# SheffieldML/GPy

Hardware: AMD Instinct MI355X
Metric: exact-GP log_lik+grad iters/sec (higher is better)
Workload: dtype f64; 1 GPU; BASELINE configs[2]: matern52 ARD exact GP, one GPRegression.parameters_changed, N=16384 D=32 Dy=1 per GPU; N=16384, D=32, kernel=matern52, ARD=True, parallelism=replicas x1

## Files before the change

### gpy_amd/csrc/gemm.hip

```cpp
#include "gemm_tile.h"
#include "internal.h"

#define LDS_OPT_IN(kernel)                                                                              \
    do {                                                                                                \
        static bool done = false;                                                                       \
        if (!done) {                                                                                    \
            (void)hipFuncSetAttribute(reinterpret_cast<const void*>(kernel),                            \
                                      hipFuncAttributeMaxDynamicSharedMemorySize, GT_LDS_BYTES);        \
            done = true;                                                                                \
        }                                                                                               \
    } while (0)

#include <algorithm>
#include <cstdlib>
#include <vector>
#define env_int(name, dflt) diag_env_int(DIAG_ENV(name), dflt)
#define LB(NW) __launch_bounds__((NW) * 64, (NW) / 2)

template <int NW, bool PRE>
__global__ LB(NW) void k_update_nt(double* __restrict__ C, long ldc,
                                                      const double* __restrict__ A, long lda,
                                                      const double* __restrict__ B, long ldb, int K, int ntc,
                                                      int row0t, int col0t, int tri, long ntiles) {
    extern __shared__ __attribute__((aligned(16))) double smem[];
    for (long bid = blockIdx.x; bid < ntiles; bid += gridDim.x) {
        int ti, tj;
        if (tri) {
            ti = (int)((sqrtf(8.0f * (float)bid + 1.0f) - 1.0f) * 0.5f);
            while ((long)ti * (ti + 1) / 2 > bid) --ti;
            while ((long)(ti + 1) * (ti + 2) / 2 <= bid) ++ti;
            tj = (int)(bid - (long)ti * (ti + 1) / 2);
        } else {
            ti = (int)(bid / ntc);
            tj = (int)(bid - (long)ti * ntc);
            if (col0t + tj > row0t + ti) continue;
        }
        d4 acc[4][GTCfg<NW>::NI];
        double* Ct = C + (long)ti * NB * ldc + (long)tj * NB;
        if (PRE) {
            gt_load_buf<NW>(Ct, ldc, acc);
            gemm_tile_128<true, true, NW, true>(A + (long)ti * NB * lda, lda, B + (long)tj * NB * ldb, ldb, K, acc, smem);
            gt_store<0, NW>(Ct, ldc, acc);
        } else {
            gt_zero<NW>(acc);
            gemm_tile_128<true, true, NW>(A + (long)ti * NB * lda, lda, B + (long)tj * NB * ldb, ldb, K, acc, smem);
            gt_store<2, NW>(Ct, ldc, acc);
        }
    }
}

__global__ __launch_bounds__(256) void k_update_nt64(double* __restrict__ C, long ldc, const double* __restrict__ A, long lda,
                                                     const double* __restrict__ B, long ldb, int K, int ntc, int row0t,
                                                     int col0t, int tri) {
    extern __shared__ __attribute__((aligned(16))) double smem[];
    const long bid = blockIdx.x >> 2;
    const int qi = (blockIdx.x >> 1) & 1, qj = blockIdx.x & 1;
    int ti, tj;
    if (tri) {
        ti = (int)((sqrtf(8.0f * (float)bid + 1.0f) - 1.0f) * 0.5f);
        while ((long)ti * (ti + 1) / 2 > bid) --ti;
        while ((long)(ti + 1) * (ti + 2) / 2 <= bid) ++ti;
        tj = (int)(bid - (long)ti * (ti + 1) / 2);
    } else {
        ti = (int)(bid / ntc);
        tj = (int)(bid - (long)ti * ntc);
        if (col0t + tj > row0t + ti) return;
    }
    d4 acc[2][2];
    double* Ct = C + ((long)ti * NB + qi * 64) * ldc + (long)tj * NB + qj * 64;
    gt64_load(Ct, ldc, acc);
    gemm_tile_64_v3<true, true, true>(A + ((long)ti * NB + qi * 64) * lda, lda, B + ((long)tj * NB + qj * 64) * ldb, ldb, K,
                                      acc, smem);
    gt64_store<0>(Ct, ldc, acc);
}

bool update_nt_uses_64(int ntr, int ntc, int row0t, int col0t) {
    static const int upd64_max = env_int("UPD64_MAX", GEMM_DEFAULT_UPD64_MAX);
    const int tri = (row0t == col0t && ntr == ntc) ? 1 : 0;
    const long nblocks = tri ? (long)ntr * (ntr + 1) / 2 : (long)ntr * ntc;
    return nblocks <= upd64_max;
}

void launch_update_nt(hipStream_t st, double* C, long ldc, const double* A, long lda, const double* B, long ldb,
                      int K, int ntr, int ntc, int row0t, int col0t) {
    if (ntr <= 0 || ntc <= 0) return;
    const int tri = (row0t == col0t && ntr == ntc) ? 1 : 0;
    const long nblocks = tri ? (long)ntr * (ntr + 1) / 2 : (long)ntr * ntc;
    if (update_nt_uses_64(ntr, ntc, row0t, col0t)) {
        hipLaunchKernelGGL(k_update_nt64, dim3((unsigned)(4 * nblocks)), dim3(256), GT64_LDS_BYTES, st, C, ldc, A, lda, B, ldb,
                           K, ntc, row0t, col0t, tri);
        return;
    }
    LDS_OPT_IN((k_update_nt<4, true>));
    hipLaunchKernelGGL((k_update_nt<4, true>), dim3((unsigned)nblocks), dim3(256), GT_LDS_BYTES, st, C, ldc, A, lda, B, ldb, K,
                       ntc, row0t, col0t, tri, nblocks);
}

#ifdef MI355GP_DIAG
__global__ LB(4) void k_update_nt_queue(double* __restrict__ A, long ld, const UpdTask* __restrict__ tasks, int ntasks,
                                        int* __restrict__ counter) {
    extern __shared__ __attribute__((aligned(16))) double smem[];
    __shared__ long s_tile;
    for (;;) {
        __syncthreads();
        if (threadIdx.x == 0) s_tile = (long)atomicAdd(counter, 1);
        __syncthreads();
        long bid = s_tile;
        int q = 0;
        while (q < ntasks && bid >= tasks[q].ntiles) bid -= tasks[q++].ntiles;
        if (q >= ntasks) return;
        const UpdTask tk = tasks[q];
        int ti = (int)((sqrtf(8.0f * (float)bid + 1.0f) - 1.0f) * 0.5f);
        while ((long)ti * (ti + 1) / 2 > bid) --ti;
        while ((long)(ti + 1) * (ti + 2) / 2 <= bid) ++ti;
        const int tj = (int)(bid - (long)ti * (ti + 1) / 2);
        d4 acc[4][GTCfg<4>::NI];
        double* Ct = A + tk.c_off + (long)ti * NB * ld + (long)tj * NB;
        const double* P = A + tk.p_off;
        gt_load_buf<4>(Ct, ld, acc);
        gemm_tile_128<true, true, 4, true>(P + (long)ti * NB * ld, ld, P + (long)tj * NB * ld, ld, tk.K, acc, smem);
        gt_store<0, 4>(Ct, ld, acc);
    }
}

void launch_update_nt_queue(hipStream_t st, double* A, long ld, const UpdTask* tasks_dev, int ntasks, int* counter, int wgs) {
    LDS_OPT_IN(k_update_nt_queue);
    hipLaunchKernelGGL(k_update_nt_queue, dim3((unsigned)wgs), dim3(256), GT_LDS_BYTES, st, A, ld, tasks_dev, ntasks, counter);
}
#endif

__host__ __device__ __forceinline__ int trtri_rows_last(int nt, int nbt) {
    const int pairs = (nt + 2 * nbt - 1) / (2 * nbt), right0 = (2 * (pairs - 1) + 1) * nbt;
    const int rows = nt - right0;
    return rows < 0 ? 0 : (rows > nbt ? nbt : rows);
}
__host__ __device__ __forceinline__ long trtri_level_tiles(int nt, int nbt) {
    const int pairs = (nt + 2 * nbt - 1) / (2 * nbt);
    return (long)(pairs - 1) * nbt * nbt + (long)nbt * trtri_rows_last(nt, nbt);
}
template <int STAGE>
__device__ __forceinline__ void trtri_map(int bid, int nt, int nbt, int& p, int& ri, int& cj) {
    const int per = nbt * nbt, pairs = (nt + 2 * nbt - 1) / (2 * nbt), full = (pairs - 1) * per;
    if (bid < full) {
        p = bid / per;
        const int rem = bid - p * per;
        if (STAGE == 1) {
            cj = rem / nbt;
            ri = rem - cj * nbt;
        } else {
            ri = nbt - 1 - rem / nbt;
            cj = rem % nbt;
        }
    } else {
        p = pairs - 1;
        const int rem = bid - full, rows = trtri_rows_last(nt, nbt);
        if (STAGE == 1) {
            cj = rem / rows;
            ri = rem - cj * rows;
        } else {
            ri = rows - 1 - rem / nbt;
            cj = rem % nbt;
        }
    }
}

template <int STAGE, int NW>
__device__ __forceinline__ void trtri_stage_tile(int bid, const double* __restrict__ L, double* __restrict__ X,
                                                 double* __restrict__ T, long ld, int nt, int nbt, double* smem) {
    int p, ri, cj;
    trtri_map<STAGE>(bid, nt, nbt, p, ri, cj);
    const int left0 = 2 * p * nbt, right0 = left0 + nbt;
    const int ti = right0 + ri, tj = left0 + cj;
    if (ti >= nt) return;
    d4 acc[4][GTCfg<NW>::NI];
// ... 462 lines not shown
```

### gpy_amd/csrc/gemm_tile.h

```cpp
#pragma once
#include "common.h"

#define GT_LDS_BYTES 73728

template <int NW>
struct GTCfg {
    static_assert(NW == 4, "the tile kernels run 4-wave workgroups");
    static constexpr int NTHR = NW * 64;
    static constexpr int NI = 4;
    static constexpr int WCOLS = NI * 16;
    static constexpr int WPR = 128 / WCOLS;
};

template <bool AK, bool BK, bool NEGA = false>
__device__ __forceinline__ void gemm_tile_128_v3(const double* __restrict__ A, long lda, const double* __restrict__ B,
                                                 long ldb, int K, d4 (&acc)[4][4], double* smem);

template <bool AK, bool BK, int NW, bool NEGA = false>
__device__ __forceinline__ void gemm_tile_128(const double* __restrict__ A, long lda,
                                              const double* __restrict__ B, long ldb, int K,
                                              d4 (&acc)[4][GTCfg<NW>::NI], double* smem) {
    gemm_tile_128_v3<AK, BK, NEGA>(A, lda, B, ldb, K, acc, smem);
}

template <int NW>
__device__ __forceinline__ void gt_zero(d4 (&acc)[4][GTCfg<NW>::NI]) {
#pragma unroll
    for (int mi = 0; mi < 4; ++mi)
#pragma unroll
        for (int ni = 0; ni < GTCfg<NW>::NI; ++ni) acc[mi][ni] = (d4){0.0, 0.0, 0.0, 0.0};
}

template <int NW>
__device__ __forceinline__ double* gt_cbase(double* C, long ldc) {
    const int t = threadIdx.x, lane = t & 63, w = t >> 6, wr = w / GTCfg<NW>::WPR, wc = w % GTCfg<NW>::WPR;
    return C + (long)(wr * 64 + (lane >> 4)) * ldc + wc * GTCfg<NW>::WCOLS + (lane & 15);
}

template <int NW>
__device__ __forceinline__ void gt_load_buf(const double* Ct, long ldc, d4 (&acc)[4][GTCfg<NW>::NI]) {
    typedef unsigned int u2 __attribute__((ext_vector_type(2)));
    const int t = threadIdx.x, lane = t & 63, w = t >> 6, wr = w / GTCfg<NW>::WPR, wc = w % GTCfg<NW>::WPR;
    __amdgpu_buffer_rsrc_t rs = __builtin_amdgcn_make_buffer_rsrc(const_cast<double*>(Ct), 0, 0x7fffffff, 0x00020000);
    const int ldb = (int)ldc * 8;
    const int voff = (wr * 64 + (lane >> 4)) * ldb + (wc * GTCfg<NW>::WCOLS + (lane & 15)) * 8;
#pragma unroll
    for (int mi = 0; mi < 4; ++mi)
#pragma unroll
        for (int r = 0; r < 4; ++r) {
            const int soff = (mi * 16 + 4 * r) * ldb;
#pragma unroll
            for (int ni = 0; ni < GTCfg<NW>::NI; ++ni) {
                const u2 v = __builtin_amdgcn_raw_buffer_load_b64(rs, voff + ni * 128, soff, 0);
                acc[mi][ni][r] = __builtin_bit_cast(double, v);
            }
        }
}

template <int NW>
__device__ __forceinline__ void gt_load_neg(const double* __restrict__ C, long ldc, d4 (&acc)[4][GTCfg<NW>::NI]) {
    const double* base = gt_cbase<NW>(const_cast<double*>(C), ldc);
#pragma unroll
    for (int mi = 0; mi < 4; ++mi)
#pragma unroll
        for (int ni = 0; ni < GTCfg<NW>::NI; ++ni)
#pragma unroll
            for (int r = 0; r < 4; ++r) acc[mi][ni][r] = -base[(long)(mi * 16 + 4 * r) * ldc + ni * 16];
}

template <int MODE, int NW>
__device__ __forceinline__ void gt_store(double* __restrict__ C, long ldc, const d4 (&acc)[4][GTCfg<NW>::NI],
                                         double alpha = 1.0, double beta = 0.0) {
    constexpr int NI = GTCfg<NW>::NI;
    double* base = gt_cbase<NW>(C, ldc);
#pragma unroll
    for (int mi = 0; mi < 4; ++mi) {
        double old[NI][4];
        if (MODE >= 2) {
#pragma unroll
            for (int ni = 0; ni < NI; ++ni)
#pragma unroll
                for (int r = 0; r < 4; ++r) old[ni][r] = base[(long)(mi * 16 + 4 * r) * ldc + ni * 16];
        }
#pragma unroll
        for (int ni = 0; ni < NI; ++ni)
#pragma unroll
            for (int r = 0; r < 4; ++r) {
                double* p = base + (long)(mi * 16 + 4 * r) * ldc + ni * 16;
                const double v = acc[mi][ni][r];
                if (MODE == 0) *p = v;
                else if (MODE == 1) *p = -v;
                else if (MODE == 2) *p = old[ni][r] - v;
                else *p = alpha * v + beta * old[ni][r];
            }
    }
}

#define GT3_SMN 132
#define GT3_OP 2176
#define GT3_LDS_BYTES (2 * 2 * GT3_OP * 8)

__device__ __forceinline__ int gt3_h(int r) { return ((r >> 1) & 7) ^ ((((r & 15) >= 4) && ((r & 15) <= 11)) ? 2 : 0); }

template <bool KC>
__device__ __forceinline__ void gt3_src_offsets(long ld, int lane, int w, int (&voff)[4]) {
#pragma unroll
    for (int ii = 0; ii < 4; ++ii) {
        const int i = 4 * w + ii;
        if (KC) {
            const int row = 8 * i + (lane >> 3), g = (lane & 7) ^ gt3_h(row);
            voff[ii] = (int)((row * ld + 2 * g) * 8);
        } else {
            voff[ii] = (int)((i * ld + 2 * lane) * 8);
        }
    }
}

template <bool KC>
__device__ __forceinline__ void gt3_issue(__amdgpu_buffer_rsrc_t rs, const int (&voff)[4], int soff, double* sdst, int w) {
#pragma unroll
    for (int ii = 0; ii < 4; ++ii) {
        const int i = 4 * w + ii;
        double* d = KC ? sdst + i * 128 : sdst + i * GT3_SMN;
        __builtin_amdgcn_raw_ptr_buffer_load_lds(rs, d, 16, voff[ii], soff, 0, 0);
    }
}

template <bool AK, bool BK, bool NEGA>
__device__ __forceinline__ void gemm_tile_128_v3(const double* __restrict__ A, long lda,
                                                 const double* __restrict__ B, long ldb, int K, d4 (&acc)[4][4],
                                                 double* smem) {
    const int t = threadIdx.x, lane = t & 63, w = t >> 6, wr = w >> 1, wc = w & 1;
    const int nk = K / 16;
    const int arow = wr * 64 + (lane & 15), bcol = wc * 64 + (lane & 15), kq = lane >> 4;
    auto rsrc = [](const double* p) {
        return __builtin_amdgcn_make_buffer_rsrc(const_cast<double*>(p), 0, 0x7fffffff, 0x00020000);
    };
    int va[4], vb[4];
    gt3_src_offsets<AK>(lda, lane, w, va);
    gt3_src_offsets<BK>(ldb, lane, w, vb);
    const long sa = AK ? 16 : 16 * lda, sb = BK ? 16 : 16 * ldb;
    int fa0[4], fb0[4];
#pragma unroll
    for (int mi = 0; mi < 4; ++mi) {
        const int r = arow + mi * 16, c = bcol + mi * 16;
        fa0[mi] = AK ? r * 16 : r;
        fb0[mi] = BK ? c * 16 : c;
    }
    const int ha = gt3_h(arow), hb = gt3_h(bcol);
    gt3_issue<AK>(rsrc(A), va, 0, smem, w);
    gt3_issue<BK>(rsrc(B), vb, 0, smem + GT3_OP, w);
    __builtin_amdgcn_s_waitcnt(0x0F70);
    __syncthreads();
    for (int kt = 0; kt < nk; ++kt) {
        const int cur = kt & 1;
        if (kt + 1 < nk) {
            double* nxt = smem + (cur ^ 1) * 2 * GT3_OP;
            gt3_issue<AK>(rsrc(A + (kt + 1) * sa), va, 0, nxt, w);
            gt3_issue<BK>(rsrc(B + (kt + 1) * sb), vb, 0, nxt + GT3_OP, w);
        }
        const double* a_s = smem + cur * 2 * GT3_OP;
        const double* b_s = a_s + GT3_OP;
#pragma unroll
        for (int e = 0; e < 2; ++e) {
            d2 af[4], bf[4];
#pragma unroll
            for (int mi = 0; mi < 4; ++mi) {
                if (AK) af[mi] = *reinterpret_cast<const d2*>(a_s + fa0[mi] + 2 * ((2 * kq + e) ^ ha));
                else af[mi] = (d2){a_s[(4 * kq + 2 * e) * GT3_SMN + fa0[mi]], a_s[(4 * kq + 2 * e + 1) * GT3_SMN + fa0[mi]]};
            }
#pragma unroll
            for (int ni = 0; ni < 4; ++ni) {
                if (BK) bf[ni] = *reinterpret_cast<const d2*>(b_s + fb0[ni] + 2 * ((2 * kq + e) ^ hb));
                else bf[ni] = (d2){b_s[(4 * kq + 2 * e) * GT3_SMN + fb0[ni]], b_s[(4 * kq + 2 * e + 1) * GT3_SMN + fb0[ni]]};
            }
#pragma unroll
            for (int s = 0; s < 2; ++s)
#pragma unroll
                for (int mi = 0; mi < 4; ++mi)
#pragma unroll
                    for (int ni = 0; ni < 4; ++ni)
                        acc[mi][ni] = mfma_f64(NEGA ? -af[mi][s] : af[mi][s], bf[ni][s], acc[mi][ni]);
        }
        __builtin_amdgcn_s_waitcnt(0x0F70);
        __syncthreads();
    }
}


template <bool AK, bool BK, bool NEGA>
__device__ __forceinline__ void gemm_tile_128_v3_multi(const double* const* __restrict__ Atab, long aoff, long lda,
                                                       const double* const* __restrict__ Btab, long boff, long ldb,
                                                       int k0, int k1, int slabs, d4 (&acc)[4][4], double* smem) {
    const int t = threadIdx.x, lane = t & 63, w = t >> 6, wr = w >> 1, wc = w & 1;
    const int nk = (k1 - k0) * slabs;
    const int arow = wr * 64 + (lane & 15), bcol = wc * 64 + (lane & 15), kq = lane >> 4;
    auto rsrc = [](const double* p) {
        return __builtin_amdgcn_make_buffer_rsrc(const_cast<double*>(p), 0, 0x7fffffff, 0x00020000);
    };
    int va[4], vb[4];
    gt3_src_offsets<AK>(lda, lane, w, va);
    gt3_src_offsets<BK>(ldb, lane, w, vb);
    const long sa = AK ? 16 : 16 * lda, sb = BK ? 16 : 16 * ldb;
    int fa0[4], fb0[4];
#pragma unroll
    for (int mi = 0; mi < 4; ++mi) {
        const int r = arow + mi * 16, c = bcol + mi * 16;
        fa0[mi] = AK ? r * 16 : r;
        fb0[mi] = BK ? c * 16 : c;
    }
    const int ha = gt3_h(arow), hb = gt3_h(bcol);
    int pk = k0, ps = 0;
    const double* Ab = Atab[pk] + aoff;
    const double* Bb = Btab[pk] + boff;
    gt3_issue<AK>(rsrc(Ab), va, 0, smem, w);
    gt3_issue<BK>(rsrc(Bb), vb, 0, smem + GT3_OP, w);
    __builtin_amdgcn_s_waitcnt(0x0F70);
    __syncthreads();
    for (int kt = 0; kt < nk; ++kt) {
        const int cur = kt & 1;
        if (kt + 1 < nk) {
            if (++ps == slabs) {
                ps = 0;
                ++pk;
                Ab = Atab[pk] + aoff;
                Bb = Btab[pk] + boff;
            }
            double* nxt = smem + (cur ^ 1) * 2 * GT3_OP;
            gt3_issue<AK>(rsrc(Ab + ps * sa), va, 0, nxt, w);
            gt3_issue<BK>(rsrc(Bb + ps * sb), vb, 0, nxt + GT3_OP, w);
        }
        const double* a_s = smem + cur * 2 * GT3_OP;
        const double* b_s = a_s + GT3_OP;
#pragma unroll
        for (int e = 0; e < 2; ++e) {
            d2 af[4], bf[4];
#pragma unroll
            for (int mi = 0; mi < 4; ++mi) {
                if (AK) af[mi] = *reinterpret_cast<const d2*>(a_s + fa0[mi] + 2 * ((2 * kq + e) ^ ha));
                else af[mi] = (d2){a_s[(4 * kq + 2 * e) * GT3_SMN + fa0[mi]], a_s[(4 * kq + 2 * e + 1) * GT3_SMN + fa0[mi]]};
            }
#pragma unroll
            for (int ni = 0; ni < 4; ++ni) {
                if (BK) bf[ni] = *reinterpret_cast<const d2*>(b_s + fb0[ni] + 2 * ((2 * kq + e) ^ hb));
                else bf[ni] = (d2){b_s[(4 * kq + 2 * e) * GT3_SMN + fb0[ni]], b_s[(4 * kq + 2 * e + 1) * GT3_SMN + fb0[ni]]};
            }
#pragma unroll
            for (int s = 0; s < 2; ++s)
#pragma unroll
                for (int mi = 0; mi < 4; ++mi)
#pragma unroll
                    for (int ni = 0; ni < 4; ++ni)
                        acc[mi][ni] = mfma_f64(NEGA ? -af[mi][s] : af[mi][s], bf[ni][s], acc[mi][ni]);
        }
        __builtin_amdgcn_s_waitcnt(0x0F70);
        __syncthreads();
    }
}

#define GT64_OP 1088
#define GT64_PAIR 136
#define GT64_LDS_BYTES (2 * 2 * GT64_OP * 8)

template <bool KC>
__device__ __forceinline__ void gt64_src_offsets(long ld, int lane, int w, int (&voff)[2]) {
#pragma unroll
    for (int ii = 0; ii < 2; ++ii) {
        const int i = 2 * w + ii;
        if (KC) {
            const int row = 8 * i + (lane >> 3), g = (lane & 7) ^ gt3_h(row);
            voff[ii] = (int)((row * ld + 2 * g) * 8);
        } else {
            voff[ii] = (int)(((2 * i + (lane >> 5)) * ld + 2 * (lane & 31)) * 8);
        }
    }
}

template <bool KC>
__device__ __forceinline__ void gt64_issue(__amdgpu_buffer_rsrc_t rs, const int (&voff)[2], double* sdst, int w) {
#pragma unroll
    for (int ii = 0; ii < 2; ++ii) {
        const int i = 2 * w + ii;
        double* d = KC ? sdst + i * 128 : sdst + i * GT64_PAIR;
        __builtin_amdgcn_raw_ptr_buffer_load_lds(rs, d, 16, voff[ii], 0, 0, 0);
    }
}

template <bool AK, bool BK, bool NEGA = false>
__device__ __forceinline__ void gemm_tile_64_v3(const double* __restrict__ A, long lda, const double* __restrict__ B,
                                                long ldb, int K, d4 (&acc)[2][2], double* smem) {
    const int t = threadIdx.x, lane = t & 63, w = t >> 6, wr = w >> 1, wc = w & 1;
    const int nk = K / 16;
    const int arow = wr * 32 + (lane & 15), bcol = wc * 32 + (lane & 15), kq = lane >> 4;
    auto rsrc = [](const double* p) {
        return __builtin_amdgcn_make_buffer_rsrc(const_cast<double*>(p), 0, 0x7fffffff, 0x00020000);
    };
    int va[2], vb[2];
    gt64_src_offsets<AK>(lda, lane, w, va);
    gt64_src_offsets<BK>(ldb, lane, w, vb);
    const long sa = AK ? 16 : 16 * lda, sb = BK ? 16 : 16 * ldb;
    int fa0[2], fb0[2];
#pragma unroll
    for (int mi = 0; mi < 2; ++mi) {
        const int r = arow + mi * 16, c = bcol + mi * 16;
        fa0[mi] = AK ? r * 16 : r;
        fb0[mi] = BK ? c * 16 : c;
    }
    const int ha = gt3_h(arow), hb = gt3_h(bcol);
    gt64_issue<AK>(rsrc(A), va, smem, w);
    gt64_issue<BK>(rsrc(B), vb, smem + GT64_OP, w);
    __builtin_amdgcn_s_waitcnt(0x0F70);
    __syncthreads();
    for (int kt = 0; kt < nk; ++kt) {
        const int cur = kt & 1;
        if (kt + 1 < nk) {
            double* nxt = smem + (cur ^ 1) * 2 * GT64_OP;
            gt64_issue<AK>(rsrc(A + (kt + 1) * sa), va, nxt, w);
            gt64_issue<BK>(rsrc(B + (kt + 1) * sb), vb, nxt + GT64_OP, w);
        }
        const double* a_s = smem + cur * 2 * GT64_OP;
        const double* b_s = a_s + GT64_OP;
#pragma unroll
        for (int e = 0; e < 2; ++e) {
            d2 af[2], bf[2];
#pragma unroll
            for (int mi = 0; mi < 2; ++mi) {
                if (AK) af[mi] = *reinterpret_cast<const d2*>(a_s + fa0[mi] + 2 * ((2 * kq + e) ^ ha));
                else af[mi] = (d2){a_s[(2 * kq + e) * GT64_PAIR + fa0[mi]], a_s[(2 * kq + e) * GT64_PAIR + 64 + fa0[mi]]};
            }
#pragma unroll
            for (int ni = 0; ni < 2; ++ni) {
                if (BK) bf[ni] = *reinterpret_cast<const d2*>(b_s + fb0[ni] + 2 * ((2 * kq + e) ^ hb));
                else bf[ni] = (d2){b_s[(2 * kq + e) * GT64_PAIR + fb0[ni]], b_s[(2 * kq + e) * GT64_PAIR + 64 + fb0[ni]]};
            }
#pragma unroll
            for (int s = 0; s < 2; ++s)
#pragma unroll
                for (int mi = 0; mi < 2; ++mi)
#pragma unroll
                    for (int ni = 0; ni < 2; ++ni)
                        acc[mi][ni] = mfma_f64(NEGA ? -af[mi][s] : af[mi][s], bf[ni][s], acc[mi][ni]);
        }
        __builtin_amdgcn_s_waitcnt(0x0F70);
        __syncthreads();
    }
}

__device__ __forceinline__ void gt64_zero(d4 (&acc)[2][2]) {
#pragma unroll
    for (int mi = 0; mi < 2; ++mi)
#pragma unroll
        for (int ni = 0; ni < 2; ++ni) acc[mi][ni] = (d4){0.0, 0.0, 0.0, 0.0};
}

__device__ __forceinline__ void gt64_load(const double* __restrict__ C, long ldc, d4 (&acc)[2][2]) {
    const int t = threadIdx.x, lane = t & 63, w = t >> 6, wr = w >> 1, wc = w & 1;
    const double* base = C + (long)(wr * 32 + (lane >> 4)) * ldc + wc * 32 + (lane & 15);
#pragma unroll
    for (int mi = 0; mi < 2; ++mi)
#pragma unroll
        for (int ni = 0; ni < 2; ++ni)
#pragma unroll
            for (int r = 0; r < 4; ++r) acc[mi][ni][r] = base[(long)(mi * 16 + 4 * r) * ldc + ni * 16];
}

template <int MODE>
__device__ __forceinline__ void gt64_store(double* __restrict__ C, long ldc, const d4 (&acc)[2][2]) {
    const int t = threadIdx.x, lane = t & 63, w = t >> 6, wr = w >> 1, wc = w & 1;
    double* base = C + (long)(wr * 32 + (lane >> 4)) * ldc + wc * 32 + (lane & 15);
#pragma unroll
    for (int mi = 0; mi < 2; ++mi)
#pragma unroll
        for (int ni = 0; ni < 2; ++ni)
#pragma unroll
            for (int r = 0; r < 4; ++r) base[(long)(mi * 16 + 4 * r) * ldc + ni * 16] = (MODE == 1) ? -acc[mi][ni][r] : acc[mi][ni][r];
}
```

### gpy_amd/csrc/grid.hip

```cpp
#include <dlfcn.h>

#include <cmath>
#include <cstdlib>
#include <cstring>
#include <functional>
#include <string>
#include <vector>

#include "../../include/mi355gp.h"
#include "../../include/mi355gp_debug.h"
#include "gemm_tile.h"
#include "internal.h"
#include "parts.h"

#define LOG_2_PI 1.8378770664093454836

#include <rccl/rccl.h>
static_assert(sizeof(ncclUniqueId) == 128, "mi355gp_grid_unique_id hands out 128-byte ids");
ncclResult_t ipcGetUniqueId(ncclUniqueId* id);
ncclResult_t ipcCommInitRank(ncclComm_t* out, int nranks, ncclUniqueId id, int rank);
ncclResult_t ipcCommSplit(ncclComm_t parent, int color, int key, ncclComm_t* out, ncclConfig_t* cfg);
ncclResult_t ipcCommDestroy(ncclComm_t comm);
ncclResult_t ipcBroadcast(const void* send, void* recv, size_t count, ncclDataType_t type, int root, ncclComm_t comm, hipStream_t st);
ncclResult_t ipcAllReduce(const void* send, void* recv, size_t count, ncclDataType_t type, ncclRedOp_t op, ncclComm_t comm, hipStream_t st);
// ... 136 lines not shown
    const int ntr = (int)(M / NB), ntc = (int)(N / NB);
    hipLaunchKernelGGL((k_grid_gemm<AK, BK>), dim3((unsigned)(ntr * ntc)), dim3(256), GT_LDS_BYTES, st, C, ldc, c_tm,
                       a.p, a.ld, a.tm, b.p, b.ld, b.tm, (int)K, ntc, (int)(nb / NB), nb, mode, pd);
}

#define GRID_ROWTAB_MAX 960
struct GridRowTab {
    int n;
    int pre[GRID_ROWTAB_MAX + 1];
};
template <bool AK, bool BK, int MODE>
__global__ __launch_bounds__(256, 2) void k_grid_gemm_multi(double* __restrict__ C, long ldc,
                                                            const double* const* __restrict__ Atab,
                                                            const double* const* __restrict__ Btab, int k0, int k1,
                                                            int ti0, int tj0, int ntc, int q, long nb, int kpred,
                                                            GridPred pd, long ldo, int tm, GridRowTab rt) {
    extern __shared__ __attribute__((aligned(16))) double smem[];
    int ti, tj;
    if (tm == 2) {
        const int bid = blockIdx.x;
        ti = (int)((sqrtf(8.0f * (float)bid + 1.0f) - 1.0f) * 0.5f);
        while ((long)ti * (ti + 1) / 2 > bid) --ti;
        while ((long)(ti + 1) * (ti + 2) / 2 <= bid) ++ti;
        tj = bid - (int)((long)ti * (ti + 1) / 2);
    } else if (rt.n > 0) {
        const int qq = q * q, p = (int)(blockIdx.x / qq), sub = (int)(blockIdx.x % qq);
        int lo = 0, hi = rt.n - 1;
        while (lo < hi) {
            const int mid = (lo + hi + 1) >> 1;
            if (rt.pre[mid] <= p) lo = mid;
            else hi = mid - 1;
        }
        ti = ti0 + lo * q + sub / q;
        tj = tj0 + (p - rt.pre[lo]) * q + sub % q;
    } else {
        ti = ti0 + blockIdx.x / ntc;
        tj = tj0 + blockIdx.x % ntc;
    }
    const int I = (ti / q) * pd.Pr + pd.pr, J = (tj / q) * pd.Pc + pd.pc;
    if (pd.on && J > I) return;
    int ks = k0;
    if (kpred >= 1 && J > ks) ks = J;
    if (kpred >= 2 && I > ks) ks = I;
    double* Ct = C + (long)ti * NB * ldc + (long)tj * NB;
    d4 acc[4][4];
    if (ks >= k1) {
        if (MODE == 0) {
            gt_zero<4>(acc);
            gt_store<0, 4>(Ct, ldc, acc);
        }
        return;
    }
    if (MODE == 0) gt_zero<4>(acc);
    else gt_load_buf<4>(Ct, ldc, acc);
    const long aoff = AK ? (long)ti * NB * ldo : (tm == 1 ? (long)(ti / q) * nb * nb + (long)(ti % q) * NB : (long)ti * NB);
    const long boff = BK ? (long)tj * NB * ldo : (tm == 1 ? (long)(tj / q) * nb * nb + (long)(tj % q) * NB : (long)tj * NB);
    gemm_tile_128_v3_multi<AK, BK, MODE == 2>(Atab, aoff, ldo, Btab, boff, ldo, ks, k1, (int)(nb / 16), acc, smem);
    gt_store<0, 4>(Ct, ldc, acc);
}

template <bool AK, bool BK, int MODE>
static void grid_gemm_multi(hipStream_t st, double* C, long ldc, const double* const* Atab, const double* const* Btab,
                            int k0, int k1, int ti0, int ti1, int tj0, int tj1, long nb, int kpred, GridPred pd,
                            long ldo = 0, int tm = 1) {
    if (ti1 <= ti0 || tj1 <= tj0 || k1 <= k0) return;
    static bool opted = false;
    if (!opted) {
        (void)hipFuncSetAttribute(reinterpret_cast<const void*>(k_grid_gemm_multi<AK, BK, MODE>),
                                  hipFuncAttributeMaxDynamicSharedMemorySize, GT_LDS_BYTES);
        opted = true;
    }
    const int q = (int)(nb / NB), ntr = (ti1 - ti0) * q, ntc = (tj1 - tj0) * q;
    long nblk = (tm == 2) ? (long)ntr * (ntr + 1) / 2 : (long)ntr * ntc;
    GridRowTab rt;
    rt.n = 0;
    if (pd.on && tm != 2 && ti1 - ti0 <= GRID_ROWTAB_MAX) {
        long tot = 0;
        int first = -1, last = -1;
        for (int li = ti0; li < ti1; ++li) {
            const long I = (long)li * pd.Pr + pd.pr;
            long m = (I >= pd.pc) ? (I - pd.pc) / pd.Pc + 1 : 0;
            long c = m - tj0;
            if (c < 0) c = 0;
            if (c > tj1 - tj0) c = tj1 - tj0;
            if (c > 0) {
                if (first < 0) first = li;
                last = li;
            }
            if (first >= 0) rt.pre[li - first] = (int)tot;
            tot += c;
        }
        if (tot == 0) return;
        rt.n = last - first + 1;
        rt.pre[rt.n] = (int)tot;
        ti0 = first;
        nblk = tot * q * q;
    }
    hipLaunchKernelGGL((k_grid_gemm_multi<AK, BK, MODE>), dim3((unsigned)nblk), dim3(256), GT_LDS_BYTES, st, C, ldc,
                       Atab, Btab, k0, k1, ti0 * q, tj0 * q, ntc, q, nb, kpred, pd, ldo ? ldo : nb, tm, rt);
}

__global__ void k_grid_fix_diag(double* __restrict__ A, long ld, long nb, long n, int ndiag,
                                const int* __restrict__ dl_r, const int* __restrict__ dl_c,
                                const int* __restrict__ dg, const double* __restrict__ noise, long noise_len,
                                double jit) {
    const long idx = (long)blockIdx.x * blockDim.x + threadIdx.x;
    if (idx >= (long)ndiag * nb) return;
    const int d = (int)(idx / nb);
    const long e = idx % nb, g = (long)dg[d] * nb + e;
    double* p = A + ((long)dl_r[d] * nb + e) * ld + (long)dl_c[d] * nb + e;
    if (g < n) *p += noise[noise_len > 1 ? g : 0] + jit;
// ... 1316 lines not shown
```

### gpy_amd/csrc/persist.hip

```cpp
#include <atomic>
#include <cstdlib>
#include <vector>

#include "chain_dev.h"
#include "gemm_tile.h"
#include "internal.h"

#define PS_NEARD 2
#define PS_MAXNT 64
#define PS_MAXT 48
#define PS_STAGE_CHUNKS 14
#define PS_STAGE_DOUBLES (PS_STAGE_CHUNKS * 128)
#define PS_LDS_BYTES ((44 * TSZ + 4 * PS_STAGE_DOUBLES) * 8)
#define PS_TIMEOUT_TICKS 50000000LL
#define PS_ARRIVE_TICKS 100000LL
#define PS_ARRIVE_ABORT (1 << 30)

#define PS_DCNT 0
#define PS_ABORT 1
#define PS_ARRIVE 2
#define PS_CNT 16
#define PS_SUB (16 + PS_MAXNT)
#define PS_DIA (16 + 2 * PS_MAXNT)
#define PS_HA (16 + 3 * PS_MAXNT)
// ... 605 lines not shown
                if (s_prog[s] >= 0 && s_wait[s] && s_cnt[nt] >= s_tk[s] + 1) {
                    pick = s; pi = s_ti[s]; pk = s_tk[s];
                    pj0 = pj1 = (pi == pk) ? pi - 1 : ((split && pi == pk + 1 && pi >= 2) ? pk - 1 : pk);
                    ptrsm = 1;
                    break;
                }
            }
        for (int o = 0; o < nmine && pick < 0; ++o) {
            const int s = s_order[o];
            const int p = s_prog[s];
            if (p == -1) continue;
            if (hot && (s_tk[s] > hotk || s_ti[s] > hoti)) continue;
            const int i = s_ti[s], k = s_tk[s];
            if (p == -2) {
                if (s_cnt[i - 1] >= i - 1 && s_pre[i]) { pick = s; pi = i; pk = i - 1; pj0 = i - 2; pj1 = i - 1; pfin = 1; break; }
                continue;
            }
            const int limit = (i == k) ? i - 1 : ((split && i == k + 1 && i >= 2) ? k - 1 : k);
            if (s_wait[s]) {
                if (s_cnt[nt] >= k + 1) { pick = s; pi = i; pk = k; pj0 = pj1 = limit; ptrsm = 1; break; }
                continue;
            }
            int jmax = s_cnt[i] < s_cnt[k] ? s_cnt[i] : s_cnt[k];
            if (jmax > limit) jmax = limit;
            if (jmax > p || p == limit) {
                pick = s; pi = i; pk = k; pj0 = p;
                pj1 = (jmax > p + kcap) ? p + kcap : (jmax > p ? jmax : p);
                ptrsm = (pj1 == limit && i >= k + 2 && s_cnt[nt] >= k + 1) ? 1 : 0;
                break;
            }
        }
        if (pick < 0) {
            if (t == 0) {
                if (idle0 == 0) idle0 = wall_clock64();
                else if (wall_clock64() - idle0 > PS_TIMEOUT_TICKS) st_flag(sync + PS_ABORT, 1);
                if (me >= own.H + own.Hh) __builtin_amdgcn_s_sleep(8);
            }
            __syncthreads();
            continue;
        }
        idle0 = 0;
        const bool subdiag = (pi == pk + 1);
        const int limit = (pi == pk) ? pi - 1 : ((split && subdiag && pi >= 2 && !pfin) ? pk - 1 : pk);
        const bool general = pi >= pk + 2;
        double* Ct = A + (long)pi * NB * ld + (long)pk * NB;
        long long* dn = (dbg && pi - pk <= 2 && (pj1 == limit)) ? dbg + 8 * nt + 4 * (3 * pi + (pi - pk)) : nullptr;
        if (dn && t == 0) dn[0] = wall_clock64();
        long long* df = (dbg && pi - pk == 3 && pj1 == limit) ? dbg + 20 * nt + 12 * pi : nullptr;
        if (df && t == 0 && pj1 > pj0) df[0] = wall_clock64();
        const bool pre = (pj1 == limit && split && subdiag && pi >= 2 && !pfin);
        const bool handover = (pj1 == limit && !general && !pre);
        if (pj1 > pj0 || (handover && subdiag)) {
            d4 acc[4][4];
            gt_load_buf<4>(Ct, ld, acc);
            if (pj1 > pj0)
                gemm_tile_128<true, true, 4, true>(A + (long)pi * NB * ld + (long)pj0 * NB, ld,
                                                   A + (long)pk * NB * ld + (long)pj0 * NB, ld, (pj1 - pj0) * NB, acc, sm);
            if (handover || subdiag) {
                __syncthreads();
                stage_put_acc(sm, acc);
                __syncthreads();
                if (handover && subdiag) stage_store_chain_order<256>(sm, hs + (long)pi * (NB * NB), t);
                else stage_store_coherent<256>(sm, Ct, ld, t);
            } else {
                gt_store<0, 4>(Ct, ld, acc);
            }
        }
        if (dn && t == 0) dn[1] = wall_clock64();
        if (df && t == 0 && pj1 > pj0) df[1] = wall_clock64();
        if (handover) {
            drain_stores();
            __syncthreads();
            if (t == 0) {
                st_flag(sync + ((pi == pk) ? PS_DIA : PS_SUB) + pi, 1);
                if (dn) dn[2] = wall_clock64();
                s_prog[pick] = -1;
            }
            --left;
        } else if (pre) {
            drain_stores();
            __syncthreads();
            if (t == 0) {
                st_flag(sync + PS_PRE + pi, 1);
                s_prog[pick] = -1;
            }
            --left;
        } else if (pj1 == limit && !ptrsm) {
            drain_stores();
            __syncthreads();
            if (t == 0) { s_prog[pick] = pj1; s_wait[pick] = 1; }
        } else if (ptrsm) {
            drain_stores();
            __syncthreads();
            if (df && t == 0) df[2] = wall_clock64();
            trsm_stage_L(A, ld, (long)pk * NB, dinv_all + (long)pk * 8 * 256, sm);
            __syncthreads();
            if (df && t == 0) df[3] = wall_clock64();
            {
                d4 Y0[8], Y1[8];
                trsm_strip2_regs(A, ld, (long)pk * NB, (long)pi * NB + 16 * w, sm, lane, Y0, Y1);
                __syncthreads();
                if (df && t == 0) df[4] = wall_clock64();
                stage_put_strips(sm, w, Y0, Y1, lane);
            }
            __syncthreads();
            stage_store_coherent<256>(sm, Ct, ld, t);
            drain_stores();
            __syncthreads();
            const bool more = split && pi == pk + 2;
            if (t == 0) {
// ... 76 lines not shown
        if (t < nt) h_cnt[t] = ld_flag(sync + PS_CNT + t);
        if (t == 64) h_cnt[nt] = ld_flag(sync + PS_DCNT);
        if (t == 65) h_cnt[nt + 1] = ld_flag(sync + PS_ABORT);
        if (t >= 128 && t < 128 + nt) h_pre[t - 128] = ld_flag(sync + PS_PRE + t - 128);
        if (t == 0) __builtin_amdgcn_fence(__ATOMIC_ACQUIRE, "agent");
        __syncthreads();
        if (h_cnt[nt + 1] != 0) return;
        const int dc = h_cnt[nt];
        bool hot = false;
        if (nreserve >= 0)
            for (int s = 0; s < nmine; ++s) hot = hot || (h_stage[s] != 3 && own.half_row(q, s) <= dc + nreserve);
        int pick = -1, pi = 0, pj0 = 0, pj1 = 0, act = 0;
        for (int s = 0; s < nmine && pick < 0; ++s) {
            const int st = h_stage[s];
            if (st == 3) continue;
            const int i = own.half_row(q, s), k = i - 2;
            if (hot && i > dc + nreserve) continue;
            if (st == 2) {
                if (h_cnt[i - 1] >= i - 1 && h_pre[i] != 0) { pick = s; pi = i; act = 3; }
                continue;
            }
            if (st == 1) {
                if (dc >= k + 1) { pick = s; pi = i; act = 2; }
                continue;
            }
            const int p = h_prog[s];
            if (p >= k) {
                pick = s; pi = i; act = (dc >= k + 1) ? 2 : 0;
                if (act == 0) { pick = -1; if (t == 0) h_stage[s] = 1; }
                continue;
            }
            int jmax = h_cnt[i] < h_cnt[k] ? h_cnt[i] : h_cnt[k];
            if (jmax > k) jmax = k;
            if (jmax > p) { pick = s; pi = i; act = 1; pj0 = p; pj1 = (jmax > p + kcap) ? p + kcap : jmax; }
        }
        if (pick < 0) {
            if (t == 0) {
                if (idle0 == 0) idle0 = wall_clock64();
                else if (wall_clock64() - idle0 > PS_TIMEOUT_TICKS) st_flag(sync + PS_ABORT, 1);
            }
            __syncthreads();
            continue;
        }
        idle0 = 0;
        const int pk = pi - 2;
        const long r0 = (long)pi * NB + 64 * h;
        long long* dn2 = (dbg && h == 0) ? dbg + 8 * nt + 4 * (3 * pi + 2) : nullptr;
        long long* dn1 = (dbg && h == 0) ? dbg + 8 * nt + 4 * (3 * pi + 1) : nullptr;
        if (act == 1) {
#pragma unroll 1
            for (int qc = 0; qc < 2; ++qc) {
                double* Cq = A + r0 * ld + (long)pk * NB + 64 * qc;
                d4 acc[2][2];
                gt64_load(Cq, ld, acc);
                gemm_tile_64_v3<true, true, true>(A + r0 * ld + (long)pj0 * NB, ld, A + ((long)pk * NB + 64 * qc) * ld + (long)pj0 * NB, ld,
                                                  (pj1 - pj0) * NB, acc, sm);
                gt64_store<0>(Cq, ld, acc);
            }
            __syncthreads();
            if (t == 0) {
                h_prog[pick] = pj1;
                if (pj1 >= pk) h_stage[pick] = 1;
            }
        } else if (act == 2) {
            if (dn2 && t == 0) dn2[0] = wall_clock64();
            drain_stores();
            __syncthreads();
            trsm_stage_L(A, ld, (long)pk * NB, dinv_all + (long)pk * 8 * 256, sm);
            __syncthreads();
            {
                const int fi = lane & 15, fk = lane >> 4;
                const double* Pa = A + (r0 + 16 * w + fi) * ld + (long)pk * NB;
                d4 P[8], Y[8];
#pragma unroll
                for (int jb = 0; jb < 8; ++jb)
#pragma unroll
                    for (int r = 0; r < 4; ++r) P[jb][r] = Pa[jb * 16 + fk + 4 * r];
                trsm_strip_core(P, Y, [sm](int jb, int k) { return sm + tix_sl(jb, k) * TSZ; }, [sm](int jb) { return sm + (28 + jb) * TSZ; },
                                lane);
                if (dn2 && t == 0) dn2[1] = wall_clock64();
                half_put_strip(img, w, Y, lane);
            }
            __syncthreads();
            half_store_coherent(img, A + r0 * ld + (long)pk * NB, ld, t);
            drain_stores();
            __syncthreads();
            if (t == 0) {
                if (__hip_atomic_fetch_add(sync + PS_HA + pi, 1, __ATOMIC_RELAXED, __HIP_MEMORY_SCOPE_AGENT) == 1)
                    st_flag(sync + PS_CNT + pi, pk + 1);
                if (dn2) dn2[2] = wall_clock64();
                h_stage[pick] = 2;
            }
        } else {
            if (dn1 && t == 0) dn1[0] = wall_clock64();
#pragma unroll 1
            for (int qc = 0; qc < 2; ++qc) {
                const double* Cq = A + r0 * ld + (long)(pi - 1) * NB + 64 * qc;
                d4 acc[2][2];
                gt64_load(Cq, ld, acc);
                gemm_tile_64_v3<true, true, true>(A + r0 * ld + (long)pk * NB, ld, A + ((long)(pi - 1) * NB + 64 * qc) * ld + (long)pk * NB, ld,
                                                  NB, acc, sm);
                half_put_acc(img, acc, qc);
            }
            __syncthreads();
            if (dn1 && t == 0) dn1[1] = wall_clock64();
            half_store_chain_order(img, hs + (long)pi * (NB * NB), h, t);
            drain_stores();
            __syncthreads();
            if (t == 0) {
                if (__hip_atomic_fetch_add(sync + PS_HB + pi, 1, __ATOMIC_RELAXED, __HIP_MEMORY_SCOPE_AGENT) == 1)
                    st_flag(sync + PS_SUB + pi, 1);
                if (dn1) dn1[2] = wall_clock64();
                h_stage[pick] = 3;
            }
            --left;
        }
        __syncthreads();
    }
}

__global__ __launch_bounds__(512, 1) void k_potrf_persist(double* __restrict__ A, long ld, int nt,
                                                          double* __restrict__ dinv_all, double* __restrict__ logsum,
                                                          int* __restrict__ info, int* __restrict__ sync, int kcap,
                                                          double* __restrict__ hs, long long* __restrict__ dbg, int test, int tune) {
    extern __shared__ __attribute__((aligned(16))) double sm[];
    if (!ps_arrive(sync, info, test == 1 ? 1 : 0)) return;
    if (test == 2 && blockIdx.x == 0) {
        if (threadIdx.x == 0) {
            st_flag(sync + PS_ABORT, 1);
            atomicMax(info, PS_ABORT_INFO);
        }
        return;
    }
    if (blockIdx.x == 0) {
        chain_workgroup(A, ld, nt, dinv_all, logsum, info, sync, hs, dbg);
        if (threadIdx.x == 0 && ld_flag(sync + PS_ABORT) != 0) atomicMax(info, PS_ABORT_INFO);
    } else {
        const int split = (tune & 4) ? 0 : 1, neard = ps_neard(tune), hdiv = ((tune >> 8) & 0xff) ? ((tune >> 8) & 0xff) : ps_hdiv(nt);
        const int nreserve = (tune & 32) ? -1 : (((tune >> 16) & 7) ? ((tune >> 16) & 7) : 3);
        const int halves = ps_halves(nt, tune);
        int H, Hh, nnear;
        ps_near_split(nt, (int)gridDim.x - 1, neard, hdiv, halves, &H, &Hh, &nnear);
        const int me = (int)blockIdx.x - 1;
        if (me >= H && me < H + Hh)
            half_workgroup(A, ld, nt, dinv_all, sync, kcap, hs, dbg, neard, hdiv, nreserve, halves, sm);
        else
            worker_workgroup(A, ld, nt, dinv_all, sync, kcap, hs, dbg, split, neard, hdiv, (tune & 1) ? 0 : 1, (tune & 2) ? 0 : 1,
                             (tune & 8) ? -1 : ((tune & 16) ? 1 : 0), nreserve,
                             ((tune >> 20) & 1) ? 1 : (((tune >> 21) & 1) ? 0 : ps_far_rowmajor(nt)), halves, sm);
    }
}

int persist_box_verdict(int set) {
    static std::atomic<int> votes[2] = {{0}, {0}};
// ... 170 lines not shown
```

Baseline: 13.89 iters/s.

## Software-pipeline LDS fragment loads and hoist negation out of MFMA inner loop

The 128 and 64 GEMM tile kernels now load the next k-half's fragments from LDS while the MFMAs for the current half run, with sched_barriers fixing the order. Global-to-LDS prefetch moves two stages ahead, into the buffer just consumed. The NEGA per-MFMA negation of A fragments is dropped; callers instead negate C on load and store with a negating mode (or negate the accumulator explicitly), so the inner loop is pure MFMA. This adds register pressure from the double fragment sets and risks correctness if any store mode or buffer reuse is mismatched.

After: 14.00 iters/s (median of 6 runs). No clear change (+0.8%).

```diff
diff --git a/gpy_amd/csrc/gemm.hip b/gpy_amd/csrc/gemm.hip
--- a/gpy_amd/csrc/gemm.hip
+++ b/gpy_amd/csrc/gemm.hip
@@ -38,9 +38,9 @@
         d4 acc[4][GTCfg<NW>::NI];
         double* Ct = C + (long)ti * NB * ldc + (long)tj * NB;
         if (PRE) {
-            gt_load_buf<NW>(Ct, ldc, acc);
-            gemm_tile_128<true, true, NW, true>(A + (long)ti * NB * lda, lda, B + (long)tj * NB * ldb, ldb, K, acc, smem);
-            gt_store<0, NW>(Ct, ldc, acc);
+            gt_load_buf<NW, true>(Ct, ldc, acc);
+            gemm_tile_128<true, true, NW>(A + (long)ti * NB * lda, lda, B + (long)tj * NB * ldb, ldb, K, acc, smem);
+            gt_store<1, NW>(Ct, ldc, acc);
         } else {
             gt_zero<NW>(acc);
             gemm_tile_128<true, true, NW>(A + (long)ti * NB * lda, lda, B + (long)tj * NB * ldb, ldb, K, acc, smem);
@@ -68,10 +68,9 @@
     }
     d4 acc[2][2];
     double* Ct = C + ((long)ti * NB + qi * 64) * ldc + (long)tj * NB + qj * 64;
-    gt64_load(Ct, ldc, acc);
-    gemm_tile_64_v3<true, true, true>(A + ((long)ti * NB + qi * 64) * lda, lda, B + ((long)tj * NB + qj * 64) * ldb, ldb, K,
-                                      acc, smem);
-    gt64_store<0>(Ct, ldc, acc);
+    gt64_load<true>(Ct, ldc, acc);
+    gemm_tile_64_v3<true, true>(A + ((long)ti * NB + qi * 64) * lda, lda, B + ((long)tj * NB + qj * 64) * ldb, ldb, K, acc, smem);
+    gt64_store<1>(Ct, ldc, acc);
 }
 
 bool update_nt_uses_64(int ntr, int ntc, int row0t, int col0t) {
@@ -117,9 +116,9 @@
         d4 acc[4][GTCfg<4>::NI];
         double* Ct = A + tk.c_off + (long)ti * NB * ld + (long)tj * NB;
         const double* P = A + tk.p_off;
-        gt_load_buf<4>(Ct, ld, acc);
-        gemm_tile_128<true, true, 4, true>(P + (long)ti * NB * ld, ld, P + (long)tj * NB * ld, ld, tk.K, acc, smem);
-        gt_store<0, 4>(Ct, ld, acc);
+        gt_load_buf<4, true>(Ct, ld, acc);
+        gemm_tile_128<true, true, 4>(P + (long)ti * NB * ld, ld, P + (long)tj * NB * ld, ld, tk.K, acc, smem);
+        gt_store<1, 4>(Ct, ld, acc);
     }
 }
 
diff --git a/gpy_amd/csrc/gemm_tile.h b/gpy_amd/csrc/gemm_tile.h
--- a/gpy_amd/csrc/gemm_tile.h
+++ b/gpy_amd/csrc/gemm_tile.h
@@ -12,15 +12,15 @@
     static constexpr int WPR = 128 / WCOLS;
 };
 
-template <bool AK, bool BK, bool NEGA = false>
+template <bool AK, bool BK>
 __device__ __forceinline__ void gemm_tile_128_v3(const double* __restrict__ A, long lda, const double* __restrict__ B,
                                                  long ldb, int K, d4 (&acc)[4][4], double* smem);
 
-template <bool AK, bool BK, int NW, bool NEGA = false>
+template <bool AK, bool BK, int NW>
 __device__ __forceinline__ void gemm_tile_128(const double* __restrict__ A, long lda,
                                               const double* __restrict__ B, long ldb, int K,
                                               d4 (&acc)[4][GTCfg<NW>::NI], double* smem) {
-    gemm_tile_128_v3<AK, BK, NEGA>(A, lda, B, ldb, K, acc, smem);
+    gemm_tile_128_v3<AK, BK>(A, lda, B, ldb, K, acc, smem);
 }
 
 template <int NW>
@@ -37,7 +37,7 @@
     return C + (long)(wr * 64 + (lane >> 4)) * ldc + wc * GTCfg<NW>::WCOLS + (lane & 15);
 }
 
-template <int NW>
+template <int NW, bool NEG = false>
 __device__ __forceinline__ void gt_load_buf(const double* Ct, long ldc, d4 (&acc)[4][GTCfg<NW>::NI]) {
     typedef unsigned int u2 __attribute__((ext_vector_type(2)));
     const int t = threadIdx.x, lane = t & 63, w = t >> 6, wr = w / GTCfg<NW>::WPR, wc = w % GTCfg<NW>::WPR;
@@ -52,7 +52,7 @@
 #pragma unroll
             for (int ni = 0; ni < GTCfg<NW>::NI; ++ni) {
                 const u2 v = __builtin_amdgcn_raw_buffer_load_b64(rs, voff + ni * 128, soff, 0);
-                acc[mi][ni][r] = __builtin_bit_cast(double, v);
+                acc[mi][ni][r] = NEG ? -__builtin_bit_cast(double, v) : __builtin_bit_cast(double, v);
             }
         }
 }
@@ -66,6 +66,14 @@
         for (int ni = 0; ni < GTCfg<NW>::NI; ++ni)
 #pragma unroll
             for (int r = 0; r < 4; ++r) acc[mi][ni][r] = -base[(long)(mi * 16 + 4 * r) * ldc + ni * 16];
+}
+
+template <int NW>
+__device__ __forceinline__ void gt_neg(d4 (&acc)[4][GTCfg<NW>::NI]) {
+#pragma unroll
+    for (int mi = 0; mi < 4; ++mi)
+#pragma unroll
+        for (int ni = 0; ni < GTCfg<NW>::NI; ++ni) acc[mi][ni] = -acc[mi][ni];
 }
 
 template <int MODE, int NW>
@@ -126,7 +134,18 @@
     }
 }
 
-template <bool AK, bool BK, bool NEGA>
+template <int NF>
+__device__ __forceinline__ void gt_mma(const d2 (&af)[NF], const d2 (&bf)[NF], d4 (&acc)[NF][NF]) {
+#pragma unroll
+    for (int s = 0; s < 2; ++s)
+#pragma unroll
+        for (int mi = 0; mi < NF; ++mi)
+#pragma unroll
+            for (int ni = 0; ni < NF; ++ni)
+                acc[mi][ni] = mfma_f64(af[mi][s], bf[ni][s], acc[mi][ni]);
+}
+
+template <bool AK, bool BK>
 __device__ __forceinline__ void gemm_tile_128_v3(const double* __restrict__ A, long lda,
                                                  const double* __restrict__ B, long ldb, int K, d4 (&acc)[4][4],
                                                  double* smem) {
@@ -148,47 +167,53 @@
         fb0[mi] = BK ? c * 16 : c;
     }
     const int ha = gt3_h(arow), hb = gt3_h(bcol);
+    auto frags = [&](const double* a_s, const double* b_s, int e, d2 (&af)[4], d2 (&bf)[4]) {
+#pragma unroll
+        for (int mi = 0; mi < 4; ++mi) {
+            if (AK) af[mi] = *reinterpret_cast<const d2*>(a_s + fa0[mi] + 2 * ((2 * kq + e) ^ ha));
+            else af[mi] = (d2){a_s[(4 * kq + 2 * e) * GT3_SMN + fa0[mi]], a_s[(4 * kq + 2 * e + 1) * GT3_SMN + fa0[mi]]};
+        }
+#pragma unroll
+        for (int ni = 0; ni < 4; ++ni) {
+            if (BK) bf[ni] = *reinterpret_cast<const d2*>(b_s + fb0[ni] + 2 * ((2 * kq + e) ^ hb));
+            else bf[ni] = (d2){b_s[(4 * kq + 2 * e) * GT3_SMN + fb0[ni]], b_s[(4 * kq + 2 * e + 1) * GT3_SMN + fb0[ni]]};
+        }
+    };
     gt3_issue<AK>(rsrc(A), va, 0, smem, w);
     gt3_issue<BK>(rsrc(B), vb, 0, smem + GT3_OP, w);
     __builtin_amdgcn_s_waitcnt(0x0F70);
     __syncthreads();
+    if (nk > 1) {
+        gt3_issue<AK>(rsrc(A + sa), va, 0, smem + 2 * GT3_OP, w);
+        gt3_issue<BK>(rsrc(B + sb), vb, 0, smem + 3 * GT3_OP, w);
+    }
+    d2 af0[4], bf0[4], af1[4], bf1[4];
+    frags(smem, smem + GT3_OP, 0, af0, bf0);
     for (int kt = 0; kt < nk; ++kt) {
         const int cur = kt & 1;
-        if (kt + 1 < nk) {
-            double* nxt = smem + (cur ^ 1) * 2 * GT3_OP;
-            gt3_issue<AK>(rsrc(A + (kt + 1) * sa), va, 0, nxt, w);
-            gt3_issue<BK>(rsrc(B + (kt + 1) * sb), vb, 0, nxt + GT3_OP, w);
-        }
-        const double* a_s = smem + cur * 2 * GT3_OP;
-        const double* b_s = a_s + GT3_OP;
-#pragma unroll
-        for (int e = 0; e < 2; ++e) {
-            d2 af[4], bf[4];
-#pragma unroll
-            for (int mi = 0; mi < 4; ++mi) {
-                if (AK) af[mi] = *reinterpret_cast<const d2*>(a_s + fa0[mi] + 2 * ((2 * kq + e) ^ ha));
-                else af[mi] = (d2){a_s[(4 * kq + 2 * e) * GT3_SMN + fa0[mi]], a_s[(4 * kq + 2 * e + 1) * GT3_SMN + fa0[mi]]};
-            }
-#pragma unroll
-            for (int ni = 0; ni < 4; ++ni) {
-                if (BK) bf[ni] = *reinterpret_cast<const d2*>(b_s + fb0[ni] + 2 * ((2 * kq + e) ^ hb));
-                else bf[ni] = (d2){b_s[(4 * kq + 2 * e) * GT3_SMN + fb0[ni]], b_s[(4 * kq + 2 * e + 1) * GT3_SMN + fb0[ni]]};
-            }
-#pragma unroll
-            for (int s = 0; s < 2; ++s)
-#pragma unroll
-                for (int mi = 0; mi < 4; ++mi)
-#pragma unroll
-                    for (int ni = 0; ni < 4; ++ni)
-                        acc[mi][ni] = mfma_f64(NEGA ? -af[mi][s] : af[mi][s], bf[ni][s], acc[mi][ni]);
-        }
+        double* a_s = smem + cur * 2 * GT3_OP;
+        double* n_s = smem + (cur ^ 1) * 2 * GT3_OP;
+        frags(a_s, a_s + GT3_OP, 1, af1, bf1);
+        __builtin_amdgcn_sched_barrier(0);
+        gt_mma<4>(af0, bf0, acc);
+        __builtin_amdgcn_sched_barrier(0);
         __builtin_amdgcn_s_waitcnt(0x0F70);
         __syncthreads();
-    }
-}
-
-
-template <bool AK, bool BK, bool NEGA>
+        __builtin_amdgcn_sched_barrier(0);
+        if (kt + 1 < nk) {
+            if (kt + 2 < nk) {
+                gt3_issue<AK>(rsrc(A + (kt + 2) * sa), va, 0, a_s, w);
+                gt3_issue<BK>(rsrc(B + (kt + 2) * sb), vb, 0, a_s + GT3_OP, w);
+            }
+            frags(n_s, n_s + GT3_OP, 0, af0, bf0);
+        }
+        __builtin_amdgcn_sched_barrier(0);
+        gt_mma<4>(af1, bf1, acc);
+    }
+}
+
+
+template <bool AK, bool BK>
 __device__ __forceinline__ void gemm_tile_128_v3_multi(const double* const* __restrict__ Atab, long aoff, long lda,
                                                        const double* const* __restrict__ Btab, long boff, long ldb,
                                                        int k0, int k1, int slabs, d4 (&acc)[4][4], double* smem) {
@@ -251,7 +276,7 @@
                 for (int mi = 0; mi < 4; ++mi)
 #pragma unroll
                     for (int ni = 0; ni < 4; ++ni)
-                        acc[mi][ni] = mfma_f64(NEGA ? -af[mi][s] : af[mi][s], bf[ni][s], acc[mi][ni]);
+                        acc[mi][ni] = mfma_f64(af[mi][s], bf[ni][s], acc[mi][ni]);
         }
         __builtin_amdgcn_s_waitcnt(0x0F70);
         __syncthreads();
@@ -286,7 +311,7 @@
     }
 }
 
-template <bool AK, bool BK, bool NEGA = false>
+template <bool AK, bool BK>
 __device__ __forceinline__ void gemm_tile_64_v3(const double* __restrict__ A, long lda, const double* __restrict__ B,
                                                 long ldb, int K, d4 (&acc)[2][2], double* smem) {
     const int t = threadIdx.x, lane = t & 63, w = t >> 6, wr = w >> 1, wc = w & 1;
@@ -307,42 +332,48 @@
         fb0[mi] = BK ? c * 16 : c;
     }
     const int ha = gt3_h(arow), hb = gt3_h(bcol);
+    auto frags = [&](const double* a_s, const double* b_s, int e, d2 (&af)[2], d2 (&bf)[2]) {
+#pragma unroll
+        for (int mi = 0; mi < 2; ++mi) {
+            if (AK) af[mi] = *reinterpret_cast<const d2*>(a_s + fa0[mi] + 2 * ((2 * kq + e) ^ ha));
+            else af[mi] = (d2){a_s[(2 * kq + e) * GT64_PAIR + fa0[mi]], a_s[(2 * kq + e) * GT64_PAIR + 64 + fa0[mi]]};
+        }
+#pragma unroll
+        for (int ni = 0; ni < 2; ++ni) {
+            if (BK) bf[ni] = *reinterpret_cast<const d2*>(b_s + fb0[ni] + 2 * ((2 * kq + e) ^ hb));
+            else bf[ni] = (d2){b_s[(2 * kq + e) * GT64_PAIR + fb0[ni]], b_s[(2 * kq + e) * GT64_PAIR + 64 + fb0[ni]]};
+        }
+    };
     gt64_issue<AK>(rsrc(A), va, smem, w);
     gt64_issue<BK>(rsrc(B), vb, smem + GT64_OP, w);
     __builtin_amdgcn_s_waitcnt(0x0F70);
     __syncthreads();
+    if (nk > 1) {
+        gt64_issue<AK>(rsrc(A + sa), va, smem + 2 * GT64_OP, w);
+        gt64_issue<BK>(rsrc(B + sb), vb, smem + 3 * GT64_OP, w);
+    }
+    d2 af0[2], bf0[2], af1[2], bf1[2];
+    frags(smem, smem + GT64_OP, 0, af0, bf0);
     for (int kt = 0; kt < nk; ++kt) {
         const int cur = kt & 1;
-        if (kt + 1 < nk) {
-            double* nxt = smem + (cur ^ 1) * 2 * GT64_OP;
-            gt64_issue<AK>(rsrc(A + (kt + 1) * sa), va, nxt, w);
-            gt64_issue<BK>(rsrc(B + (kt + 1) * sb), vb, nxt + GT64_OP, w);
-        }
-        const double* a_s = smem + cur * 2 * GT64_OP;
-        const double* b_s = a_s + GT64_OP;
-#pragma unroll
-        for (int e = 0; e < 2; ++e) {
-            d2 af[2], bf[2];
-#pragma unroll
-            for (int mi = 0; mi < 2; ++mi) {
-                if (AK) af[mi] = *reinterpret_cast<const d2*>(a_s + fa0[mi] + 2 * ((2 * kq + e) ^ ha));
-                else af[mi] = (d2){a_s[(2 * kq + e) * GT64_PAIR + fa0[mi]], a_s[(2 * kq + e) * GT64_PAIR + 64 + fa0[mi]]};
-            }
-#pragma unroll
-            for (int ni = 0; ni < 2; ++ni) {
-                if (BK) bf[ni] = *reinterpret_cast<const d2*>(b_s + fb0[ni] + 2 * ((2 * kq + e) ^ hb));
-                else bf[ni] = (d2){b_s[(2 * kq + e) * GT64_PAIR + fb0[ni]], b_s[(2 * kq + e) * GT64_PAIR + 64 + fb0[ni]]};
-            }
-#pragma unroll
-            for (int s = 0; s < 2; ++s)
-#pragma unroll
-                for (int mi = 0; mi < 2; ++mi)
-#pragma unroll
-                    for (int ni = 0; ni < 2; ++ni)
-                        acc[mi][ni] = mfma_f64(NEGA ? -af[mi][s] : af[mi][s], bf[ni][s], acc[mi][ni]);
-        }
+        double* a_s = smem + cur * 2 * GT64_OP;
+        double* n_s = smem + (cur ^ 1) * 2 * GT64_OP;
+        frags(a_s, a_s + GT64_OP, 1, af1, bf1);
+        __builtin_amdgcn_sched_barrier(0);
+        gt_mma<2>(af0, bf0, acc);
+        __builtin_amdgcn_sched_barrier(0);
         __builtin_amdgcn_s_waitcnt(0x0F70);
         __syncthreads();
+        __builtin_amdgcn_sched_barrier(0);
+        if (kt + 1 < nk) {
+            if (kt + 2 < nk) {
+                gt64_issue<AK>(rsrc(A + (kt + 2) * sa), va, a_s, w);
+                gt64_issue<BK>(rsrc(B + (kt + 2) * sb), vb, a_s + GT64_OP, w);
+            }
+            frags(n_s, n_s + GT64_OP, 0, af0, bf0);
+        }
+        __builtin_amdgcn_sched_barrier(0);
+        gt_mma<2>(af1, bf1, acc);
     }
 }
 
@@ -353,6 +384,7 @@
         for (int ni = 0; ni < 2; ++ni) acc[mi][ni] = (d4){0.0, 0.0, 0.0, 0.0};
 }
 
+template <bool NEG = false>
 __device__ __forceinline__ void gt64_load(const double* __restrict__ C, long ldc, d4 (&acc)[2][2]) {
     const int t = threadIdx.x, lane = t & 63, w = t >> 6, wr = w >> 1, wc = w & 1;
     const double* base = C + (long)(wr * 32 + (lane >> 4)) * ldc + wc * 32 + (lane & 15);
@@ -361,7 +393,17 @@
 #pragma unroll
         for (int ni = 0; ni < 2; ++ni)
 #pragma unroll
-            for (int r = 0; r < 4; ++r) acc[mi][ni][r] = base[(long)(mi * 16 + 4 * r) * ldc + ni * 16];
+            for (int r = 0; r < 4; ++r) {
+                const double v = base[(long)(mi * 16 + 4 * r) * ldc + ni * 16];
+                acc[mi][ni][r] = NEG ? -v : v;
+            }
+}
+
+__device__ __forceinline__ void gt64_neg(d4 (&acc)[2][2]) {
+#pragma unroll
+    for (int mi = 0; mi < 2; ++mi)
+#pragma unroll
+        for (int ni = 0; ni < 2; ++ni) acc[mi][ni] = -acc[mi][ni];
 }
 
 template <int MODE>
diff --git a/gpy_amd/csrc/grid.hip b/gpy_amd/csrc/grid.hip
--- a/gpy_amd/csrc/grid.hip
+++ b/gpy_amd/csrc/grid.hip
@@ -212,11 +212,11 @@
         return;
     }
     if (MODE == 0) gt_zero<4>(acc);
-    else gt_load_buf<4>(Ct, ldc, acc);
+    else gt_load_buf<4, MODE == 2>(Ct, ldc, acc);
     const long aoff = AK ? (long)ti * NB * ldo : (tm == 1 ? (long)(ti / q) * nb * nb + (long)(ti % q) * NB : (long)ti * NB);
     const long boff = BK ? (long)tj * NB * ldo : (tm == 1 ? (long)(tj / q) * nb * nb + (long)(tj % q) * NB : (long)tj * NB);
-    gemm_tile_128_v3_multi<AK, BK, MODE == 2>(Atab, aoff, ldo, Btab, boff, ldo, ks, k1, (int)(nb / 16), acc, smem);
-    gt_store<0, 4>(Ct, ldc, acc);
+    gemm_tile_128_v3_multi<AK, BK>(Atab, aoff, ldo, Btab, boff, ldo, ks, k1, (int)(nb / 16), acc, smem);
+    gt_store<MODE == 2 ? 1 : 0, 4>(Ct, ldc, acc);
 }
 
 template <bool AK, bool BK, int MODE>
diff --git a/gpy_amd/csrc/persist.hip b/gpy_amd/csrc/persist.hip
--- a/gpy_amd/csrc/persist.hip
+++ b/gpy_amd/csrc/persist.hip
@@ -681,10 +681,11 @@
         const bool handover = (pj1 == limit && !general && !pre);
         if (pj1 > pj0 || (handover && subdiag)) {
             d4 acc[4][4];
-            gt_load_buf<4>(Ct, ld, acc);
+            gt_load_buf<4, true>(Ct, ld, acc);
             if (pj1 > pj0)
-                gemm_tile_128<true, true, 4, true>(A + (long)pi * NB * ld + (long)pj0 * NB, ld,
-                                                   A + (long)pk * NB * ld + (long)pj0 * NB, ld, (pj1 - pj0) * NB, acc, sm);
+                gemm_tile_128<true, true, 4>(A + (long)pi * NB * ld + (long)pj0 * NB, ld,
+                                             A + (long)pk * NB * ld + (long)pj0 * NB, ld, (pj1 - pj0) * NB, acc, sm);
+            gt_neg<4>(acc);
             if (handover || subdiag) {
                 __syncthreads();
                 stage_put_acc(sm, acc);
@@ -867,10 +868,10 @@
             for (int qc = 0; qc < 2; ++qc) {
                 double* Cq = A + r0 * ld + (long)pk * NB + 64 * qc;
                 d4 acc[2][2];
-                gt64_load(Cq, ld, acc);
-                gemm_tile_64_v3<true, true, true>(A + r0 * ld + (long)pj0 * NB, ld, A + ((long)pk * NB + 64 * qc) * ld + (long)pj0 * NB, ld,
-                                                  (pj1 - pj0) * NB, acc, sm);
-                gt64_store<0>(Cq, ld, acc);
+                gt64_load<true>(Cq, ld, acc);
+                gemm_tile_64_v3<true, true>(A + r0 * ld + (long)pj0 * NB, ld, A + ((long)pk * NB + 64 * qc) * ld + (long)pj0 * NB, ld,
+                                            (pj1 - pj0) * NB, acc, sm);
+                gt64_store<1>(Cq, ld, acc);
             }
             __syncthreads();
             if (t == 0) {
@@ -912,9 +913,10 @@
             for (int qc = 0; qc < 2; ++qc) {
                 const double* Cq = A + r0 * ld + (long)(pi - 1) * NB + 64 * qc;
                 d4 acc[2][2];
-                gt64_load(Cq, ld, acc);
-                gemm_tile_64_v3<true, true, true>(A + r0 * ld + (long)pk * NB, ld, A + ((long)(pi - 1) * NB + 64 * qc) * ld + (long)pk * NB, ld,
-                                                  NB, acc, sm);
+                gt64_load<true>(Cq, ld, acc);
+                gemm_tile_64_v3<true, true>(A + r0 * ld + (long)pk * NB, ld, A + ((long)(pi - 1) * NB + 64 * qc) * ld + (long)pk * NB, ld,
+                                            NB, acc, sm);
+                gt64_neg(acc);
                 half_put_acc(img, acc, qc);
             }
             __syncthreads();
```
